# somepago/DCR

Measured on AMD Instinct MI355X. Metric: sd21_256px_finetune_imgs_per_sec, higher is better.
Workload: dtype bf16; 1 GPU; model=sd2.1-unet-865M-random-init, global_batch=16, resolution=256, seq_len=77, parallelism=dp1, optimizer=fused_adamw

## Files before the change

### dcr_amd/ops/adamw.py

```python
from __future__ import annotations

from typing import Iterable, List, Tuple

import torch

from . import use_hip, require_hip, count_dispatch

QBLOCK = 256
FP8_MAX = 448.0
STATE_FORMAT = {"state_bits": 8, "qblock": QBLOCK, "codec": "e4m3fn_absmax",
                "second_moment": "sqrt"}


def _nblocks(numel: int) -> int:
    return (numel + QBLOCK - 1) // QBLOCK


def _sqrt_rn(x: torch.Tensor) -> torch.Tensor:
    return x.double().sqrt().float()


@torch.no_grad()
def quantize_blockwise(x: torch.Tensor) -> Tuple[torch.Tensor, torch.Tensor]:
    dev = x.device
    x = x.detach().reshape(-1).float()
    nb = _nblocks(x.numel())
    xp = torch.zeros(nb * QBLOCK, dtype=torch.float32, device=dev)
    xp[: x.numel()] = x
    xp = xp.view(nb, QBLOCK)
    absmax = xp.abs().amax(dim=1)
    scale = torch.full_like(absmax, FP8_MAX).div(absmax)
    ok = torch.isfinite(scale)
    scale = torch.where(ok, scale, torch.zeros_like(scale))
    y = (xp * scale[:, None]).clamp_(-FP8_MAX, FP8_MAX)
# ... 76 lines not shown
            n = p.numel()
            sl = self.flat_param[offset : offset + n]
            gl = self.flat_grad[offset : offset + n]
            if (p.data.dim() == 4 and not p.data.is_contiguous()
                    and p.data.is_contiguous(
                        memory_format=torch.channels_last)):
                K, C, Hh, Ww = p.data.shape
                sl.copy_(p.data.permute(0, 2, 3, 1).reshape(-1))
                p.data = sl.view(K, Hh, Ww, C).permute(0, 3, 1, 2)
                self._grad_views.append(
                    gl.view(K, Hh, Ww, C).permute(0, 3, 1, 2))
            else:
                sl.copy_(p.data.reshape(-1))
                p.data = sl.view_as(p.data)
                self._grad_views.append(gl.view_as(p.data))
            self.offsets.append(offset)
            offset += n
        self.numel = total
        self._view_of = {id(p): v for p, v in zip(self.params, self._grad_views)}
        self._gathered: set = set()
        if self.master is not None:
            self.master.copy_(self.flat_param.float())

        self.hyper = None
        if device_state and device.type == "cuda":
            self.hyper = torch.tensor([lr, 1, 1, 1, 1, 1, 0, 0],
                                      dtype=torch.float32, device=device)

    def zero_grad(self, set_to_none: bool = False):
        if len(self._gathered) != len(self.params):
            self.flat_grad.zero_()
            self._skipped_zero = False
        else:
            self._skipped_zero = True
        self._gathered.clear()
        for p in self.params:
            p.grad = None

    def _ensure_cold_slices(self):
        if not getattr(self, "_skipped_zero", False):
            return
        if len(self._gathered) == len(self.params):
            return
        stale = [self._view_of[id(p)] for p in self.params
                 if id(p) not in self._gathered]
        if stale:
            torch._foreach_zero_(stale)
        self._skipped_zero = False

    @torch.no_grad()
    def gather_grads(self, params=None):
        copy_d, copy_s, add_d, add_s = [], [], [], []
        for p in (params if params is not None else self.params):
            g = p.grad
            if g is None:
                continue
            view = self._view_of[id(p)]
            if g.dtype != view.dtype:
                g = g.to(view.dtype)
            if id(p) in self._gathered:
                add_d.append(view)
                add_s.append(g)
            else:
                copy_d.append(view)
                copy_s.append(g)
                self._gathered.add(id(p))
            p.grad = None
        if copy_d:
            torch._foreach_copy_(copy_d, copy_s)
        if add_d:
            torch._foreach_add_(add_d, add_s)

    @torch.no_grad()
    def step(self, lr: float | None = None):
        self.gather_grads()
        self._ensure_cold_slices()
        if lr is not None:
            self.lr = lr
        self.step_count += 1
        t = self.step_count
        if self.state_bits == 8:
            self._step8(t)
            return
        if use_hip(self.flat_param):
            m = require_hip("adamw")
            if m is not None:
                count_dispatch('adamw')
                if self.master is not None:
                    m.adamw_step_bf16(
                        self.flat_param, self.flat_grad, self.master,
                        self.exp_avg, self.exp_avg_sq, self.lr, self.beta1,
# ... 67 lines not shown
            ts = (self.exp_avg, self.exp_avg_sq)
        return sum(t.numel() * t.element_size() for t in ts)

    @torch.no_grad()
    def step_dev(self, lr: float | None = None):
        assert self.hyper is not None, "built without device_state=True"
        self.gather_grads()
        self._ensure_cold_slices()
        if lr is not None and lr != self.lr:
            self.lr = lr
            self.hyper[0].fill_(lr)
        self.step_count += 1
        m = require_hip("adamw")
        count_dispatch('adamw_dev')
        m.adamw_step_dev(self.flat_param, self.flat_grad, self.master,
                         self.exp_avg, self.exp_avg_sq, self.hyper,
                         self.beta1, self.beta2, self.eps, self.weight_decay,
                         self.max_grad_norm)

    @torch.no_grad()
    def clip_grad_norm_(self, max_norm: float) -> torch.Tensor:
        self.gather_grads()
        self._ensure_cold_slices()
        norm = torch.linalg.vector_norm(self.flat_grad, dtype=torch.float32)
        scale = max_norm / (norm + 1e-6)
        if float(norm) > max_norm:
            self.flat_grad.mul_(scale.to(self.flat_grad.dtype))
        return norm

    def state_dict(self):
        if self.state_bits == 8:
            d = {
                "step": self.step_count,
                "lr": self.lr,
                "flat_param": self.flat_param,
                "exp_avg_q": self.exp_avg_q,
                "exp_avg_absmax": self.exp_avg_absmax,
                "exp_avg_sq_q": self.exp_avg_sq_q,
                "exp_avg_sq_absmax": self.exp_avg_sq_absmax,
                "format": dict(STATE_FORMAT),
            }
            if self.master is not None:
                d["master"] = self.master
            return d
        d = {
            "step": self.step_count,
            "lr": self.lr,
            "exp_avg": self.exp_avg,
            "exp_avg_sq": self.exp_avg_sq,
            "flat_param": self.flat_param,
        }
# ... 81 lines not shown
```

### dcr_amd/ops/build.py

```python
from __future__ import annotations

import os
import shutil
from pathlib import Path

HERE = Path(__file__).resolve().parent
HIP_DIR = HERE / "hip"
BUILD_DIR = HERE / "_build"
TARGET = HERE / "_dcr_hip.so"

SOURCES = [
    HIP_DIR / "bindings.cpp",
    HIP_DIR / "norms.hip",
    HIP_DIR / "norms_nhwc.hip",
    HIP_DIR / "elementwise.hip",
    HIP_DIR / "reduce.hip",
    HIP_DIR / "adamw8.hip",
    HIP_DIR / "attention.hip",
    HIP_DIR / "conv_nhwc.hip",
    HIP_DIR / "conv_nhwc_bwd.hip",
    HIP_DIR / "gemm.hip",
    HIP_DIR / "maxsim.hip",
    HIP_DIR / "splitsim.hip",
    HIP_DIR / "topk_sim.hip",
]


def build_extension(verbose: bool = False, force: bool = False) -> Path:
    os.environ.setdefault("PYTORCH_ROCM_ARCH", "gfx950")
    os.environ.setdefault("MAX_JOBS", str(min(16, os.cpu_count() or 4)))
    from torch.utils import cpp_extension

    BUILD_DIR.mkdir(parents=True, exist_ok=True)
    if force:
        for f in BUILD_DIR.glob("*"):
            if f.is_file():
                f.unlink()

    cpp_extension.load(
        name="_dcr_hip",
        sources=[str(s) for s in SOURCES],
        build_directory=str(BUILD_DIR),
        extra_cflags=["-O3"],
        extra_cuda_cflags=["-O3"],
# ... 14 lines not shown
```

### dcr_amd/ops/hip/bindings.cpp

```cpp

#include <torch/extension.h>
#include <ATen/cuda/CUDAContext.h>

#include <climits>
#include <cstdint>
#include <limits>

#include "dcr_launchers.h"

using namespace dcr;

namespace {

DType dtype_of(const at::Tensor& t) {
  switch (t.scalar_type()) {
    case at::kFloat: return DT_F32;
    case at::kHalf: return DT_F16;
    case at::kBFloat16: return DT_BF16;
    default: TORCH_CHECK(false, "dcr_hip: unsupported dtype ", t.scalar_type());
  }
}

hipStream_t cur_stream() {
  return at::cuda::getCurrentCUDAStream().stream();
}

at::Tensor as_f32(const at::Tensor& t) {
  return t.scalar_type() == at::kFloat ? t.contiguous()
                                       : t.to(at::kFloat).contiguous();
// ... 225 lines not shown

void adamw_step(at::Tensor p, at::Tensor g, at::Tensor m, at::Tensor v,
                double lr, double beta1, double beta2, double eps, double wd,
                int64_t step) {
  TORCH_CHECK(p.is_cuda() && p.scalar_type() == at::kFloat,
              "adamw: fp32 flat params expected");
  TORCH_CHECK(p.is_contiguous() && g.is_contiguous() && m.is_contiguous() &&
              v.is_contiguous());
  adamw_launch(p.data_ptr<float>(), g.data_ptr<float>(), m.data_ptr<float>(),
               v.data_ptr<float>(), p.numel(), (float)lr, (float)beta1,
               (float)beta2, (float)eps, (float)wd, step, cur_stream());
}

void adamw_step_bf16(at::Tensor p, at::Tensor g, at::Tensor master,
                     at::Tensor m, at::Tensor v, double lr, double beta1,
                     double beta2, double eps, double wd, int64_t step) {
  TORCH_CHECK(p.is_cuda() && p.scalar_type() == at::kBFloat16);
  TORCH_CHECK(master.scalar_type() == at::kFloat);
  TORCH_CHECK(p.is_contiguous() && g.is_contiguous() && master.is_contiguous());
  adamw_bf16_launch(p.data_ptr(), g.data_ptr(), master.data_ptr<float>(),
                    m.data_ptr<float>(), v.data_ptr<float>(), p.numel(),
                    (float)lr, (float)beta1, (float)beta2, (float)eps,
                    (float)wd, step, cur_stream());
}

void adamw_step_dev(at::Tensor p, at::Tensor g, c10::optional<at::Tensor> master,
                    at::Tensor m, at::Tensor v, at::Tensor hyper, double beta1,
                    double beta2, double eps, double wd, double max_norm) {
  TORCH_CHECK(hyper.is_cuda() && hyper.scalar_type() == at::kFloat &&
              hyper.numel() == 8 && hyper.is_contiguous());
  TORCH_CHECK(p.is_contiguous() && g.is_contiguous());
  const bool bf16 = p.scalar_type() == at::kBFloat16;
  float* mp = nullptr;
  if (bf16) {
    TORCH_CHECK(master.has_value() && master->scalar_type() == at::kFloat,
                "bf16 device-state adamw needs the fp32 master");
    mp = master->data_ptr<float>();
  } else {
    TORCH_CHECK(p.scalar_type() == at::kFloat);
  }
  adamw_dev_launch(bf16 ? 1 : 0, p.data_ptr(), g.data_ptr(), mp,
                   m.data_ptr<float>(), v.data_ptr<float>(), p.numel(),
                   (float)beta1, (float)beta2, (float)eps, (float)wd,
                   (float)max_norm, hyper.data_ptr<float>(), cur_stream());
}

// ... 684 lines not shown
  mod.def("attn_fwd_d512", &attn_fwd_d512);
  mod.def("attn_bwd_gen", &attn_bwd_gen);
  mod.def("attn_fwd_v2", &attn_fwd_v2);
  mod.def("attn_fwd_v3", &attn_fwd_v3);
  mod.def("attn_fwd_v4", &attn_fwd_v4);
  mod.def("attn_bwd", &attn_bwd);
  mod.def("attn_bwd_v4", &attn_bwd_v4);
  mod.def("mfma_probe", &mfma_probe);
  mod.def("groupnorm_silu_fwd", &groupnorm_silu_fwd);
  mod.def("groupnorm_silu_bwd", &groupnorm_silu_bwd);
  mod.def("groupnorm_silu_nhwc_fwd", &groupnorm_silu_nhwc_fwd);
  mod.def("groupnorm_silu_nhwc_bwd", &groupnorm_silu_nhwc_bwd);
  mod.def("layernorm_fwd", &layernorm_fwd);
  mod.def("layernorm_bwd", &layernorm_bwd, py::arg("dy"), py::arg("x"),
          py::arg("w"), py::arg("mean"), py::arg("rstd"),
          py::arg("blocks") = 0);
  mod.def("colsum", &colsum);
  mod.def("colsum_grouped", &colsum_grouped);
  mod.def("geglu_fwd", &geglu_fwd);
  mod.def("geglu_bwd", &geglu_bwd);
  mod.def("adamw_step", &adamw_step);
  mod.def("adamw_step_bf16", &adamw_step_bf16);
  mod.def("adamw_step_dev", &adamw_step_dev);
  mod.def("adamw8_step", &adamw8_step, py::arg("p"), py::arg("g"),
          py::arg("exp_avg_q"), py::arg("exp_avg_absmax"),
          py::arg("exp_avg_sq_q"), py::arg("exp_avg_sq_absmax"), py::arg("lr"),
          py::arg("beta1"), py::arg("beta2"), py::arg("eps"), py::arg("wd"),
          py::arg("step"));
  mod.def("adamw8_step_bf16", &adamw8_step_bf16, py::arg("p"), py::arg("g"),
          py::arg("master"), py::arg("exp_avg_q"), py::arg("exp_avg_absmax"),
          py::arg("exp_avg_sq_q"), py::arg("exp_avg_sq_absmax"), py::arg("lr"),
          py::arg("beta1"), py::arg("beta2"), py::arg("eps"), py::arg("wd"),
          py::arg("step"));
  mod.def("add_noise", &add_noise);
  mod.def("get_velocity", &get_velocity);
  mod.def("cfg_combine", &cfg_combine);
  mod.def("lincomb", &lincomb);
}
```

### dcr_amd/ops/hip/dcr_launchers.h

```cpp
#pragma once

#include <hip/hip_runtime.h>

namespace dcr {

enum DType { DT_F32 = 0, DT_F16 = 1, DT_BF16 = 2 };

void gn_fwd_launch(DType dt, const void* x, const void* w, const void* b,
                   bool w_f32, void* y, float* mean, float* rstd, int NG,
                   int G, int Cg, int HW, float eps, bool silu, hipStream_t s);
void gn_bwd_launch(DType dt, const void* dy, const void* x, const void* w,
                   const void* b, bool w_f32, const float* mean,
                   const float* rstd, void* dx, float* dw, float* db, int NG,
                   int G, int Cg, int HW, bool silu, hipStream_t s);
void ln_fwd_launch(DType dt, const void* x, const void* w, const void* b,
                   bool w_f32, void* y, float* mean, float* rstd, long M,
                   int N, float eps, hipStream_t s);
void ln_bwd_launch(DType dt, const void* dy, const void* x, const void* w,
                   bool w_f32, const float* mean, const float* rstd, void* dx,
                   float* dw, float* db, long M, int N, hipStream_t s);
int ln_bwd_v2_blocks(long M, int N);
void ln_bwd_v2_launch(DType dt, const void* dy, const void* x, const void* w,
                      bool w_f32, const float* mean, const float* rstd,
                      void* dx, float* slab, void* dwdb, int blocks, long M,
// ... 5 lines not shown
                        int N, int R, int C, int G, float eps, bool silu,
                        hipStream_t s);
void gn_nhwc_bwd_launch(DType dt, const void* dy, const void* x, const void* w,
                        const void* b, bool w_f32, const float* mean,
                        const float* rstd, float* ws, void* dx, void* dwdb,
                        int N, int R, int C, int G, bool silu,
                        hipStream_t s);

int colsum_chunks(int dt, long groups, long rows_per_group, int C, int cap);
void colsum_launch(DType dt, const void* x, float* slab, void* out_n, void* out,
                   long groups, long rows_per_group, int C, int chunks,
                   hipStream_t s);

void geglu_fwd_launch(DType dt, const void* x, void* y, long M, long N,
                      hipStream_t s);
void geglu_bwd_launch(DType dt, const void* dy, const void* x, void* dx,
                      long M, long N, hipStream_t s);
void adamw_launch(float* p, const float* g, float* m, float* v, long n,
                  float lr, float b1, float b2, float eps, float wd, long step,
                  hipStream_t s);
void adamw_bf16_launch(void* p, const void* g, float* master, float* m,
                       float* v, long n, float lr, float b1, float b2,
                       float eps, float wd, long step, hipStream_t s);
void adamw_dev_launch(int bf16, void* p, const void* g, float* master,
                      float* m, float* v, long n, float b1, float b2,
                      float eps, float wd, float max_norm, float* hyper,
                      hipStream_t s);
void adamw8_launch(int bf16, void* p, const void* g, float* master,
                   unsigned char* mq, float* mabs, unsigned char* rq,
                   float* rabs, long n, double lr, double b1, double b2,
                   double eps, double wd, long step, hipStream_t s);
void sched_launch(DType dt, int mode, const void* x0, const void* noise,
                  const float* ac, const long* t, void* out, long per_sample,
                  long total, hipStream_t s);
void cfg_launch(DType dt, const void* eu, const void* et, void* out, float s_,
                long total, hipStream_t s);
void lincomb_launch(DType dt, const void* X, const void* Y, const void* Z,
                    void* out, float a, float b, float c, long total,
                    hipStream_t s);

void attn_fwd_launch(const void* q, const void* k, const void* v, void* o,
                     float* lse, int BH, int Lq, int Lk, int H, float scale,
                     bool causal, hipStream_t s);
void attn_fwd_v2_launch(const void* q, const void* k, const void* v, void* o,
                        float* lse, int BH, int Lq, int Lk, int H, float scale,
                        bool causal, hipStream_t s);
// ... 75 lines not shown
```

### dcr_amd/ops/hip/elementwise.hip

```cpp

#include "dcr_common.h"

using namespace dcr;

template <typename T>
__global__ void geglu_fwd_kernel(const T* __restrict__ x, T* __restrict__ y,
                                 long M, long N) {
  const long nvec = M * N / 4;
  for (long i = (long)blockIdx.x * blockDim.x + threadIdx.x; i < nvec;
       i += (long)gridDim.x * blockDim.x) {
    long e = i * 4;
    long row = e / N, col = e % N;
    const T* base = x + row * 2 * N;
    f32x4 a = load4<T>(base + col);
    f32x4 g = load4<T>(base + N + col);
    f32x4 o;
    o.x = a.x * gelu_erf(g.x);
    o.y = a.y * gelu_erf(g.y);
    o.z = a.z * gelu_erf(g.z);
    o.w = a.w * gelu_erf(g.w);
    store4<T>(y + row * N + col, o);
  }
}

template <typename T>
__global__ void geglu_bwd_kernel(const T* __restrict__ dy, const T* __restrict__ x,
                                 T* __restrict__ dx, long M, long N) {
  const long nvec = M * N / 4;
  for (long i = (long)blockIdx.x * blockDim.x + threadIdx.x; i < nvec;
       i += (long)gridDim.x * blockDim.x) {
    long e = i * 4;
    long row = e / N, col = e % N;
    const T* base = x + row * 2 * N;
    T* dbase = dx + row * 2 * N;
    f32x4 a = load4<T>(base + col);
    f32x4 g = load4<T>(base + N + col);
    f32x4 d = load4<T>(dy + row * N + col);
    f32x4 da, dg;
    da.x = d.x * gelu_erf(g.x); dg.x = d.x * a.x * dgelu_erf(g.x);
    da.y = d.y * gelu_erf(g.y); dg.y = d.y * a.y * dgelu_erf(g.y);
    da.z = d.z * gelu_erf(g.z); dg.z = d.z * a.z * dgelu_erf(g.z);
    da.w = d.w * gelu_erf(g.w); dg.w = d.w * a.w * dgelu_erf(g.w);
    store4<T>(dbase + col, da);
    store4<T>(dbase + N + col, dg);
  }
}

__global__ void adamw_kernel(float* __restrict__ p, const float* __restrict__ g,
                             float* __restrict__ m, float* __restrict__ v,
                             long n, float lr, float beta1, float beta2,
                             float eps, float wd, float inv_bc1, float inv_bc2) {
  const long nvec = n / 4;
  for (long i = (long)blockIdx.x * blockDim.x + threadIdx.x; i < nvec;
       i += (long)gridDim.x * blockDim.x) {
    long e = i * 4;
    f32x4 pv = load4<float>(p + e);
    f32x4 gv = load4<float>(g + e);
    f32x4 mv = load4<float>(m + e);
    f32x4 vv = load4<float>(v + e);
#pragma unroll
    for (int k = 0; k < 4; ++k) {
      float gg = (&gv.x)[k];
      float mm = beta1 * (&mv.x)[k] + (1.f - beta1) * gg;
      float vvk = beta2 * (&vv.x)[k] + (1.f - beta2) * gg * gg;
      (&mv.x)[k] = mm;
      (&vv.x)[k] = vvk;
      float denom = sqrtf(vvk * inv_bc2) + eps;
      float upd = (mm * inv_bc1) / denom + wd * (&pv.x)[k];
      (&pv.x)[k] -= lr * upd;
    }
    store4<float>(p + e, pv);
    store4<float>(m + e, mv);
    store4<float>(v + e, vv);
  }
  long tail = nvec * 4 + (long)blockIdx.x * blockDim.x + threadIdx.x;
  if (tail < n) {
    float gg = g[tail];
    float mm = beta1 * m[tail] + (1.f - beta1) * gg;
    float vvk = beta2 * v[tail] + (1.f - beta2) * gg * gg;
    m[tail] = mm; v[tail] = vvk;
    float denom = sqrtf(vvk * inv_bc2) + eps;
    p[tail] -= lr * ((mm * inv_bc1) / denom + wd * p[tail]);
  }
}

__global__ void adamw_bf16_kernel(__hip_bfloat16* __restrict__ p,
                                  const __hip_bfloat16* __restrict__ g,
                                  float* __restrict__ master,
                                  float* __restrict__ m, float* __restrict__ v,
                                  long n, float lr, float beta1, float beta2,
                                  float eps, float wd, float inv_bc1,
                                  float inv_bc2) {
  const long nvec = n / 4;
  for (long i = (long)blockIdx.x * blockDim.x + threadIdx.x; i < nvec;
       i += (long)gridDim.x * blockDim.x) {
    long e = i * 4;
    f32x4 gv = load4<__hip_bfloat16>(g + e);
    f32x4 pv = load4<float>(master + e);
    f32x4 mv = load4<float>(m + e);
    f32x4 vv = load4<float>(v + e);
#pragma unroll
    for (int kk = 0; kk < 4; ++kk) {
      float gg = (&gv.x)[kk];
      float mm = beta1 * (&mv.x)[kk] + (1.f - beta1) * gg;
      float vvk = beta2 * (&vv.x)[kk] + (1.f - beta2) * gg * gg;
      (&mv.x)[kk] = mm;
      (&vv.x)[kk] = vvk;
      float denom = sqrtf(vvk * inv_bc2) + eps;
      (&pv.x)[kk] -= lr * ((mm * inv_bc1) / denom + wd * (&pv.x)[kk]);
    }
    store4<float>(master + e, pv);
    store4<float>(m + e, mv);
    store4<float>(v + e, vv);
    store4<__hip_bfloat16>(p + e, pv);
  }
  long tail = nvec * 4 + (long)blockIdx.x * blockDim.x + threadIdx.x;
  if (tail < n) {
    float gg = to_f32<__hip_bfloat16>(g[tail]);
    float mm = beta1 * m[tail] + (1.f - beta1) * gg;
    float vvk = beta2 * v[tail] + (1.f - beta2) * gg * gg;
    m[tail] = mm; v[tail] = vvk;
    float denom = sqrtf(vvk * inv_bc2) + eps;
    float pv = master[tail] - lr * ((mm * inv_bc1) / denom + wd * master[tail]);
    master[tail] = pv;
    p[tail] = from_f32<__hip_bfloat16>(pv);
  }
}

template <typename T, int MODE>
__global__ void sched_kernel(const T* __restrict__ x0, const T* __restrict__ noise,
                             const float* __restrict__ ac, const long* __restrict__ t,
                             T* __restrict__ out, long per_sample, long total) {
  const long nvec = total / 4;
  for (long i = (long)blockIdx.x * blockDim.x + threadIdx.x; i < nvec;
       i += (long)gridDim.x * blockDim.x) {
    long e = i * 4;
    long bidx = e / per_sample;
    float a = ac[t[bidx]];
    float sa = sqrtf(a), sb = sqrtf(1.f - a);
    f32x4 xa = load4<T>(x0 + e);
    f32x4 xb = load4<T>(noise + e);
// ... 206 lines not shown
  switch (dt) {
    case DT_F32: hipLaunchKernelGGL((geglu_fwd_kernel<float>), grid, block, 0, s, (const float*)x, (float*)y, M, N); break;
    case DT_F16: hipLaunchKernelGGL((geglu_fwd_kernel<__half>), grid, block, 0, s, (const __half*)x, (__half*)y, M, N); break;
    case DT_BF16: hipLaunchKernelGGL((geglu_fwd_kernel<__hip_bfloat16>), grid, block, 0, s, (const __hip_bfloat16*)x, (__hip_bfloat16*)y, M, N); break;
  }
}

void geglu_bwd_launch(DType dt, const void* dy, const void* x, void* dx,
                      long M, long N, hipStream_t s) {
  dim3 grid(ew_blocks(M * N / 4)), block(256);
  switch (dt) {
    case DT_F32: hipLaunchKernelGGL((geglu_bwd_kernel<float>), grid, block, 0, s, (const float*)dy, (const float*)x, (float*)dx, M, N); break;
    case DT_F16: hipLaunchKernelGGL((geglu_bwd_kernel<__half>), grid, block, 0, s, (const __half*)dy, (const __half*)x, (__half*)dx, M, N); break;
    case DT_BF16: hipLaunchKernelGGL((geglu_bwd_kernel<__hip_bfloat16>), grid, block, 0, s, (const __hip_bfloat16*)dy, (const __hip_bfloat16*)x, (__hip_bfloat16*)dx, M, N); break;
  }
}

void adamw_launch(float* p, const float* g, float* m, float* v, long n,
                  float lr, float b1, float b2, float eps, float wd, long step,
                  hipStream_t s) {
  float bc1 = 1.f - powf(b1, (float)step);
  float bc2 = 1.f - powf(b2, (float)step);
  dim3 grid(ew_blocks(n / 4)), block(256);
  hipLaunchKernelGGL(adamw_kernel, grid, block, 0, s, p, g, m, v, n, lr, b1, b2,
                     eps, wd, 1.f / bc1, 1.f / bc2);
}

void adamw_bf16_launch(void* p, const void* g, float* master, float* m,
                       float* v, long n, float lr, float b1, float b2,
                       float eps, float wd, long step, hipStream_t s) {
  float bc1 = 1.f - powf(b1, (float)step);
  float bc2 = 1.f - powf(b2, (float)step);
  dim3 grid(ew_blocks(n / 4)), block(256);
  hipLaunchKernelGGL(adamw_bf16_kernel, grid, block, 0, s,
                     (__hip_bfloat16*)p, (const __hip_bfloat16*)g, master, m, v,
                     n, lr, b1, b2, eps, wd, 1.f / bc1, 1.f / bc2);
}

void adamw_dev_launch(int bf16, void* p, const void* g, float* master,
                      float* m, float* v, long n, float b1, float b2,
                      float eps, float wd, float max_norm, float* hyper,
                      hipStream_t s) {
  dim3 grid(ew_blocks(n / 4)), block(256);
  if (bf16)
    hipLaunchKernelGGL((gnormsq_kernel<__hip_bfloat16>), grid, block, 0, s,
                       (const __hip_bfloat16*)g, n, hyper + 6);
  else
    hipLaunchKernelGGL((gnormsq_kernel<float>), grid, block, 0, s,
                       (const float*)g, n, hyper + 6);
  hipLaunchKernelGGL(adamw_prologue_kernel, dim3(1), dim3(1), 0, s, hyper,
                     b1, b2, max_norm);
  if (bf16)
    hipLaunchKernelGGL(adamw_bf16_dev_kernel, grid, block, 0, s,
                       (__hip_bfloat16*)p, (const __hip_bfloat16*)g, master,
                       m, v, n, b1, b2, eps, wd, hyper);
  else
    hipLaunchKernelGGL(adamw_dev_kernel, grid, block, 0, s, (float*)p,
                       (const float*)g, m, v, n, b1, b2, eps, wd, hyper);
}
// ... 53 lines not shown
```

### dcr_amd/parallel/ddp.py

```python
from __future__ import annotations

from typing import List, Optional

import torch.distributed as dist

from ..ops.adamw import FusedAdamW
from . import dist as dist_utils


class _Bucket:
    __slots__ = ("start", "end", "params", "pending", "work")

    def __init__(self, start: int, end: int, params: list):
        self.start = start
        self.end = end
        self.params = params
        self.pending = len(params)
        self.work = None


class GradBucketAllReduce:

    def __init__(self, optimizer: FusedAdamW, bucket_mb: float = 64.0,
                 process_group: Optional[object] = None):
# ... 19 lines not shown
        for p, off in reversed(runs):
            n = p.numel()
            if cur_start is None:
                cur_params, cur_start, cur_end = [p], off, off + n
            else:
                cur_params.append(p)
                cur_start = off
            if cur_end - cur_start >= bucket_elems:
                self._push_bucket(cur_start, cur_end, cur_params)
                cur_params, cur_start, cur_end = [], None, None
        if cur_params:
            self._push_bucket(cur_start, cur_end, cur_params)

        for p in self.opt.params:
            p.register_post_accumulate_grad_hook(self._hook)

    def _push_bucket(self, start, end, params):
        b = _Bucket(start, end, list(params))
        self.buckets.append(b)
        for p in params:
            self._param_bucket[id(p)] = b

    def _launch(self, b: _Bucket):
        self.opt.gather_grads(b.params)
        sl = self.opt.flat_grad[b.start:b.end]
        b.work = dist.all_reduce(sl, group=self.pg, async_op=True)

    def _hook(self, param):
        if not self.require_backward_grad_sync:
            return
        b = self._param_bucket[id(param)]
        b.pending -= 1
        if b.pending == 0:
            self._launch(b)

    def finalize(self):
        self.opt.gather_grads()
        self.opt._ensure_cold_slices()
        if not self._enabled or not self.require_backward_grad_sync:
            self._reset()
            return
        for b in self.buckets:
            if b.work is None and b.pending > 0:
                self._launch(b)
        launched = any(b.work is not None for b in self.buckets)
        for b in self.buckets:
            if b.work is not None:
                b.work.wait()
        if launched and self.world > 1:
            self.opt.flat_grad.div_(self.world)
        self._reset()

    def _reset(self):
        for b in self.buckets:
            b.pending = len(b.params)
            b.work = None
```

### dcr_amd/train/trainer.py

```python
from __future__ import annotations

import os
import random
import time
from pathlib import Path
from typing import Optional

import numpy as np
import torch
import torch.nn.functional as F
from torch.utils.data import DataLoader, WeightedRandomSampler
from torch.utils.data.distributed import DistributedSampler

from ..data import (HashTokenizer, ObjectAttributeDataset, SyntheticImageDataset,
                    collate_fn, load_tokenizer)
from ..models import (AutoencoderKL, CLIPTextModel, UNet2DConditionModel,
                      UNetConfig, model_configs)
from ..models.model_io import save_pipeline_index
from ..ops.adamw import FusedAdamW
from ..parallel import GradBucketAllReduce, dist as dist_utils
from ..schedulers import DDPMScheduler
from ..utils import Tracker
from ..utils.profiler import PhaseProfiler
from .config import TrainConfig, get_lr
# ... 275 lines not shown

            if self.noise_scheduler.prediction_type == "epsilon":
                target = noise
            elif self.noise_scheduler.prediction_type == "v_prediction":
                target = self.noise_scheduler.get_velocity(latents, noise, timesteps)
            else:
                raise ValueError(self.noise_scheduler.prediction_type)

        loss = F.mse_loss(model_pred.float(), target.float(), reduction="mean")
        accum = cfg.gradient_accumulation_steps
        bwd_loss = loss / accum if accum > 1 else loss
        with self.prof.phase("backward"):
            if self.scaler is not None:
                self.scaler.scale(bwd_loss).backward()
            else:
                bwd_loss.backward()

        if sync_gradients:
            with self.prof.phase("optimizer"):
                self.ddp.finalize()
                grads_finite = True
                if self.scaler is not None:
                    inv = 1.0 / self.scaler.get_scale()
                    self.optimizer.flat_grad.mul_(inv)
                    grads_finite = bool(
                        torch.isfinite(self.optimizer.flat_grad).all())
                if grads_finite:
                    lr_step = get_lr(cfg, self.global_step, self.world)
                    if self.optimizer.hyper is not None:
                        self.optimizer.step_dev(lr=lr_step)
                    else:
                        self.optimizer.clip_grad_norm_(cfg.max_grad_norm)
                        self.optimizer.step(lr=lr_step)
                    if self.scaler is not None:
                        self._finite_streak += 1
                        if self._finite_streak >= 2000:
                            self.scaler.update(self.scaler.get_scale() * 2.0)
                            self._finite_streak = 0
                        else:
                            self.scaler.update(self.scaler.get_scale())
                else:
                    self._finite_streak = 0
                    self.scaler.update(self.scaler.get_scale() * 0.5)
                self.optimizer.zero_grad()
            self.global_step += 1
        return loss.detach()

    def fit(self, max_steps: Optional[int] = None, sample_fn=None):
        try:
            self._fit_inner(max_steps, sample_fn)
        except Exception:
            import traceback
            print(f"rank {self.rank}: training failed\n{traceback.format_exc()}",
                  flush=True)
            if dist_utils.is_dist():
                import torch.distributed as dist
# ... 96 lines not shown
```

Baseline: 265.9 imgs/sec.

## Fuse grad gather with sum-of-squares and fold clip coefficient into AdamW

Replaces the per-tensor foreach copy of gradients into the flat arena with one table-driven HIP kernel that also produces per-chunk squared-norm partials. A single-block finalize kernel turns these into the norm and clip coefficient on the device, and new clip-aware AdamW kernels read that coefficient. This removes the separate vector_norm pass, the host sync from float(norm), and the separate scaling multiply. The cost is extra bookkeeping to invalidate cached partials whenever the arena is written, plus a pinned host upload of the offset table on every step.

```diff
diff --git a/dcr_amd/ops/adamw.py b/dcr_amd/ops/adamw.py
--- a/dcr_amd/ops/adamw.py
+++ b/dcr_amd/ops/adamw.py
@@ -1,15 +1,23 @@
 from __future__ import annotations
 
+import os
 from typing import Iterable, List, Tuple
 
 import torch
 
 from . import use_hip, require_hip, count_dispatch
+
+GATHER_CH = 16384
+GATHER_GRID = 0
 
 QBLOCK = 256
 FP8_MAX = 448.0
 STATE_FORMAT = {"state_bits": 8, "qblock": QBLOCK, "codec": "e4m3fn_absmax",
                 "second_moment": "sqrt"}
+
+
+def fused_grad_tail_enabled() -> bool:
+    return os.environ.get("DCR_FUSED_GRAD_TAIL", "1") != "0"
 
 
 def _nblocks(numel: int) -> int:
@@ -132,12 +140,19 @@
         if self.master is not None:
             self.master.copy_(self.flat_param.float())
 
+        self._nvb_all = sum((p.numel() + GATHER_CH - 1) // GATHER_CH
+                            for p in self.params)
+        self._partials = None
+        self._norm_rec = None
+        self._sumsq_valid = False
+
         self.hyper = None
         if device_state and device.type == "cuda":
             self.hyper = torch.tensor([lr, 1, 1, 1, 1, 1, 0, 0],
                                       dtype=torch.float32, device=device)
 
     def zero_grad(self, set_to_none: bool = False):
+        self.arena_written()
         if len(self._gathered) != len(self.params):
             self.flat_grad.zero_()
             self._skipped_zero = False
@@ -155,11 +170,30 @@
         stale = [self._view_of[id(p)] for p in self.params
                  if id(p) not in self._gathered]
         if stale:
+            self.arena_written()
             torch._foreach_zero_(stale)
         self._skipped_zero = False
 
-    @torch.no_grad()
-    def gather_grads(self, params=None):
+    def arena_written(self):
+        self._sumsq_valid = False
+
+    def _native_tail(self):
+        if not self.flat_grad.is_cuda or not fused_grad_tail_enabled():
+            return None
+        if torch.cuda.is_current_stream_capturing():
+            return None
+        return require_hip("grad_tail")
+
+    def _get_partials(self) -> torch.Tensor:
+        if self._partials is None:
+            self._partials = torch.empty(
+                max(self._nvb_all, 1), dtype=torch.float32,
+                device=self.flat_grad.device)
+        return self._partials
+
+    @torch.no_grad()
+    def gather_grads(self, params=None, sumsq: bool = True):
+        m = self._native_tail()
         copy_d, copy_s, add_d, add_s = [], [], [], []
         for p in (params if params is not None else self.params):
             g = p.grad
@@ -176,7 +210,23 @@
                 copy_s.append(g)
                 self._gathered.add(id(p))
             p.grad = None
-        if copy_d:
+        if copy_d or add_d:
+            self.arena_written()
+        if copy_d and m is not None:
+            fused = (sumsq and params is None and not add_d
+                     and len(copy_d) == len(self.params))
+            rejected = m.grad_gather(
+                self.flat_grad, copy_d, copy_s,
+                self._get_partials() if fused else None,
+                GATHER_CH, GATHER_GRID)
+            count_dispatch('grad_gather')
+            for i in rejected:
+                count_dispatch('grad_gather_fallback')
+                copy_d[i].copy_(copy_s[i])
+            self._sumsq_valid = fused and not rejected
+        elif copy_d:
+            if self.flat_grad.is_cuda:
+                count_dispatch('grad_gather_foreach')
             torch._foreach_copy_(copy_d, copy_s)
         if add_d:
             torch._foreach_add_(add_d, add_s)
@@ -290,11 +340,57 @@
     def clip_grad_norm_(self, max_norm: float) -> torch.Tensor:
         self.gather_grads()
         self._ensure_cold_slices()
+        if self.flat_grad.is_cuda:
+            count_dispatch('grad_norm_aten')
         norm = torch.linalg.vector_norm(self.flat_grad, dtype=torch.float32)
         scale = max_norm / (norm + 1e-6)
         if float(norm) > max_norm:
+            self.arena_written()
             self.flat_grad.mul_(scale.to(self.flat_grad.dtype))
         return norm
+
+    def _norm_record(self, m, max_norm: float) -> torch.Tensor:
+        if self._norm_rec is None:
+            self._norm_rec = torch.zeros(3, dtype=torch.float32,
+                                         device=self.flat_grad.device)
+        partials = self._get_partials()
+        if not self._sumsq_valid:
+            count_dispatch('grad_sumsq')
+            m.grad_sumsq(self.flat_grad, self._grad_views, partials,
+                         GATHER_CH, GATHER_GRID)
+            self._sumsq_valid = True
+        count_dispatch('grad_norm_finalize')
+        m.sumsq_finalize(partials, self._nvb_all, float(max_norm),
+                         self._norm_rec)
+        return self._norm_rec
+
+    @torch.no_grad()
+    def clip_and_step(self, max_norm: float, lr: float | None = None) -> torch.Tensor:
+        m = self._native_tail() if self.state_bits == 32 else None
+        if m is None:
+            norm = self.clip_grad_norm_(max_norm)
+            self.step(lr=lr)
+            return norm
+        self.gather_grads()
+        self._ensure_cold_slices()
+        rec = self._norm_record(m, max_norm)
+        if lr is not None:
+            self.lr = lr
+        self.step_count += 1
+        count_dispatch('adamw')
+        count_dispatch('adamw_clip')
+        if self.master is not None:
+            m.adamw_step_bf16_clip(
+                self.flat_param, self.flat_grad, self.master, self.exp_avg,
+                self.exp_avg_sq, self.lr, self.beta1, self.beta2, self.eps,
+                self.weight_decay, self.step_count, rec)
+        else:
+            m.adamw_step_clip(
+                self.flat_param, self.flat_grad, self.exp_avg,
+                self.exp_avg_sq, self.lr, self.beta1, self.beta2, self.eps,
+                self.weight_decay, self.step_count, rec)
+        self.arena_written()
+        return rec[1]
 
     def state_dict(self):
         if self.state_bits == 8:
diff --git a/dcr_amd/ops/build.py b/dcr_amd/ops/build.py
--- a/dcr_amd/ops/build.py
+++ b/dcr_amd/ops/build.py
@@ -20,6 +20,7 @@
     HIP_DIR / "conv_nhwc.hip",
     HIP_DIR / "conv_nhwc_bwd.hip",
     HIP_DIR / "gemm.hip",
+    HIP_DIR / "grad_tail.hip",
     HIP_DIR / "maxsim.hip",
     HIP_DIR / "splitsim.hip",
     HIP_DIR / "topk_sim.hip",
diff --git a/dcr_amd/ops/hip/bindings.cpp b/dcr_amd/ops/hip/bindings.cpp
--- a/dcr_amd/ops/hip/bindings.cpp
+++ b/dcr_amd/ops/hip/bindings.cpp
@@ -4,7 +4,9 @@
 
 #include <climits>
 #include <cstdint>
+#include <cstring>
 #include <limits>
+#include <vector>
 
 #include "dcr_launchers.h"
 
@@ -276,6 +278,170 @@
                     m.data_ptr<float>(), v.data_ptr<float>(), p.numel(),
                     (float)lr, (float)beta1, (float)beta2, (float)eps,
                     (float)wd, step, cur_stream());
+}
+
+namespace {
+
+void gt_check_arena(const at::Tensor& arena, int64_t ch) {
+  TORCH_CHECK(arena.is_cuda() && arena.dim() == 1 && arena.is_contiguous(),
+              "grad tail: the arena must be a flat contiguous GPU tensor");
+  TORCH_CHECK(arena.scalar_type() == at::kBFloat16 ||
+              arena.scalar_type() == at::kFloat,
+              "grad tail: bf16 or fp32 arena expected");
+  TORCH_CHECK(ch >= 8 && ch % 8 == 0 && ch <= (1 << 24),
+              "grad tail: chunk must be a multiple of 8 elements, got ", ch);
+}
+
+int64_t gt_view_offset(const at::Tensor& arena, const at::Tensor& view) {
+  TORCH_CHECK(view.scalar_type() == arena.scalar_type() &&
+              view.device() == arena.device() &&
+              view.is_non_overlapping_and_dense(),
+              "grad tail: not a dense view of the arena");
+  const int64_t es = arena.element_size();
+  const int64_t byte_off = (const char*)view.data_ptr() - (const char*)arena.data_ptr();
+  TORCH_CHECK(byte_off >= 0 && byte_off % es == 0 &&
+              byte_off / es + view.numel() <= arena.numel(),
+              "grad tail: view outside the arena");
+  return byte_off / es;
+}
+
+bool gt_qualifies(const at::Tensor& g, const at::Tensor& view) {
+  if (!g.defined() || g.device() != view.device() ||
+      g.scalar_type() != view.scalar_type() || g.sizes() != view.sizes() ||
+      !g.is_non_overlapping_and_dense())
+    return false;
+  for (int64_t d = 0; d < g.dim(); ++d)
+    if (g.size(d) > 1 && g.stride(d) != view.stride(d)) return false;
+  return reinterpret_cast<uintptr_t>(g.data_ptr()) % g.element_size() == 0;
+}
+
+at::Tensor gt_upload(const at::Tensor& arena, const std::vector<int64_t>& rows) {
+  auto host = at::empty({(int64_t)rows.size()},
+                        at::TensorOptions().dtype(at::kLong).pinned_memory(true));
+  std::memcpy(host.data_ptr<int64_t>(), rows.data(), rows.size() * sizeof(int64_t));
+  auto dev = at::empty({(int64_t)rows.size()}, arena.options().dtype(at::kLong));
+  dev.copy_(host, true);
+  return dev;
+}
+
+float* gt_partials(const c10::optional<at::Tensor>& partials,
+                   const at::Tensor& arena, int64_t nvb) {
+  if (!partials.has_value()) return nullptr;
+  TORCH_CHECK(partials->is_cuda() && partials->device() == arena.device() &&
+              partials->scalar_type() == at::kFloat &&
+              partials->is_contiguous() && partials->numel() >= nvb,
+              "grad tail: partials must hold ", nvb, " floats on the GPU");
+  return partials->data_ptr<float>();
+}
+
+}
+
+std::vector<int64_t> grad_gather(at::Tensor arena, std::vector<at::Tensor> views,
+                                 std::vector<at::Tensor> grads,
+                                 c10::optional<at::Tensor> partials,
+                                 int64_t ch, int64_t grid) {
+  gt_check_arena(arena, ch);
+  TORCH_CHECK(views.size() == grads.size(), "grad_gather: list lengths differ");
+  std::vector<int64_t> rows, rejected;
+  rows.reserve(4 * views.size());
+  int64_t nvb = 0;
+  for (size_t i = 0; i < views.size(); ++i) {
+    if (!gt_qualifies(grads[i], views[i])) {
+      rejected.push_back((int64_t)i);
+      continue;
+    }
+    const int64_t n = views[i].numel();
+    if (n == 0) continue;
+    const int64_t off = gt_view_offset(arena, views[i]);
+    rows.push_back((int64_t)reinterpret_cast<uintptr_t>(grads[i].data_ptr()));
+    rows.push_back(off);
+    rows.push_back(n);
+    rows.push_back(nvb);
+    nvb += (n + ch - 1) / ch;
+  }
+  if (rows.empty()) return rejected;
+  float* pp = gt_partials(partials, arena, nvb);
+  auto table = gt_upload(arena, rows);
+  grad_gather_launch(dtype_of(arena), (const long*)table.data_ptr<int64_t>(),
+                     (int)(rows.size() / 4), nvb, arena.data_ptr(), pp, (int)ch,
+                     grad_gather_grid(nvb, (int)grid), true,
+                     cur_stream());
+  return rejected;
+}
+
+int64_t grad_sumsq(at::Tensor arena, std::vector<at::Tensor> views,
+                   at::Tensor partials, int64_t ch, int64_t grid) {
+  gt_check_arena(arena, ch);
+  std::vector<int64_t> rows;
+  rows.reserve(4 * views.size());
+  int64_t nvb = 0;
+  for (const auto& v : views) {
+    const int64_t n = v.numel();
+    if (n == 0) continue;
+    const int64_t off = gt_view_offset(arena, v);
+    rows.push_back((int64_t)reinterpret_cast<uintptr_t>(
+        (const char*)arena.data_ptr() + off * arena.element_size()));
+    rows.push_back(off);
+    rows.push_back(n);
+    rows.push_back(nvb);
+    nvb += (n + ch - 1) / ch;
+  }
+  float* pp = gt_partials(partials, arena, nvb);
+  if (rows.empty()) return 0;
+  auto table = gt_upload(arena, rows);
+  grad_gather_launch(dtype_of(arena), (const long*)table.data_ptr<int64_t>(),
+                     (int)(rows.size() / 4), nvb, arena.data_ptr(), pp, (int)ch,
+                     grad_gather_grid(nvb, (int)grid), false,
+                     cur_stream());
+  return nvb;
+}
+
+void sumsq_finalize(at::Tensor partials, int64_t nvb, double max_norm,
+                    at::Tensor rec) {
+  TORCH_CHECK(partials.is_cuda() && partials.scalar_type() == at::kFloat &&
+              partials.is_contiguous() && nvb >= 0 && partials.numel() >= nvb,
+              "sumsq_finalize: partials must hold nvb floats on the GPU");
+  TORCH_CHECK(rec.is_cuda() && rec.scalar_type() == at::kFloat &&
+              rec.is_contiguous() && rec.numel() == 3,
+              "sumsq_finalize: rec must be float[3] on the GPU");
+  sumsq_finalize_launch(partials.data_ptr<float>(), nvb, (float)max_norm,
+                        rec.data_ptr<float>(), cur_stream());
+}
+
+static void gt_check_rec(const at::Tensor& rec, const at::Tensor& p) {
+  TORCH_CHECK(rec.is_cuda() && rec.device() == p.device() &&
+              rec.scalar_type() == at::kFloat && rec.is_contiguous() &&
+              rec.numel() == 3, "adamw_clip: rec must be float[3] on the GPU");
+}
+
+void adamw_step_clip(at::Tensor p, at::Tensor g, at::Tensor m, at::Tensor v,
+                     double lr, double beta1, double beta2, double eps,
+                     double wd, int64_t step, at::Tensor rec) {
+  TORCH_CHECK(p.is_cuda() && p.scalar_type() == at::kFloat &&
+              g.scalar_type() == at::kFloat && g.numel() == p.numel(),
+              "adamw_clip: fp32 flat params and grads expected");
+  TORCH_CHECK(p.is_contiguous() && g.is_contiguous() && m.is_contiguous() &&
+              v.is_contiguous());
+  gt_check_rec(rec, p);
+  adamw_clip_launch(p.data_ptr<float>(), g.data_ptr<float>(),
+                    m.data_ptr<float>(), v.data_ptr<float>(), p.numel(),
+                    (float)lr, (float)beta1, (float)beta2, (float)eps,
+                    (float)wd, step, rec.data_ptr<float>(), cur_stream());
+}
+
+void adamw_step_bf16_clip(at::Tensor p, at::Tensor g, at::Tensor master,
+                          at::Tensor m, at::Tensor v, double lr, double beta1,
+                          double beta2, double eps, double wd, int64_t step,
+                          at::Tensor rec) {
+  TORCH_CHECK(p.is_cuda() && p.scalar_type() == at::kBFloat16 &&
+              g.scalar_type() == at::kBFloat16 && g.numel() == p.numel());
+  TORCH_CHECK(master.scalar_type() == at::kFloat);
+  TORCH_CHECK(p.is_contiguous() && g.is_contiguous() && master.is_contiguous());
+  gt_check_rec(rec, p);
+  adamw_bf16_clip_launch(p.data_ptr(), g.data_ptr(), master.data_ptr<float>(),
+                         m.data_ptr<float>(), v.data_ptr<float>(), p.numel(),
+                         (float)lr, (float)beta1, (float)beta2, (float)eps,
+                         (float)wd, step, rec.data_ptr<float>(), cur_stream());
 }
 
 void adamw_step_dev(at::Tensor p, at::Tensor g, c10::optional<at::Tensor> master,
@@ -1006,6 +1172,14 @@
   mod.def("adamw_step", &adamw_step);
   mod.def("adamw_step_bf16", &adamw_step_bf16);
   mod.def("adamw_step_dev", &adamw_step_dev);
+  mod.def("adamw_step_clip", &adamw_step_clip);
+  mod.def("adamw_step_bf16_clip", &adamw_step_bf16_clip);
+  mod.def("grad_gather", &grad_gather, py::arg("arena"), py::arg("views"),
+          py::arg("grads"), py::arg("partials") = py::none(),
+          py::arg("ch") = 16384, py::arg("grid") = 0);
+  mod.def("grad_sumsq", &grad_sumsq, py::arg("arena"), py::arg("views"),
+          py::arg("partials"), py::arg("ch") = 16384, py::arg("grid") = 0);
+  mod.def("sumsq_finalize", &sumsq_finalize);
   mod.def("adamw8_step", &adamw8_step, py::arg("p"), py::arg("g"),
           py::arg("exp_avg_q"), py::arg("exp_avg_absmax"),
           py::arg("exp_avg_sq_q"), py::arg("exp_avg_sq_absmax"), py::arg("lr"),
diff --git a/dcr_amd/ops/hip/dcr_launchers.h b/dcr_amd/ops/hip/dcr_launchers.h
--- a/dcr_amd/ops/hip/dcr_launchers.h
+++ b/dcr_amd/ops/hip/dcr_launchers.h
@@ -51,6 +51,19 @@
 void adamw_bf16_launch(void* p, const void* g, float* master, float* m,
                        float* v, long n, float lr, float b1, float b2,
                        float eps, float wd, long step, hipStream_t s);
+void adamw_clip_launch(float* p, float* g, float* m, float* v, long n,
+                       float lr, float b1, float b2, float eps, float wd,
+                       long step, const float* rec, hipStream_t s);
+void adamw_bf16_clip_launch(void* p, void* g, float* master, float* m,
+                            float* v, long n, float lr, float b1, float b2,
+                            float eps, float wd, long step, const float* rec,
+                            hipStream_t s);
+int grad_gather_grid(long nvb, int grid_req);
+void grad_gather_launch(DType dt, const long* table, int nparams, long nvb,
+                        void* arena, float* partials, int ch, int grid,
+                        bool store, hipStream_t s);
+void sumsq_finalize_launch(const float* partials, long nvb, float max_norm,
+                           float* rec, hipStream_t s);
 void adamw_dev_launch(int bf16, void* p, const void* g, float* master,
                       float* m, float* v, long n, float b1, float b2,
                       float eps, float wd, float max_norm, float* hyper,
diff --git a/dcr_amd/ops/hip/elementwise.hip b/dcr_amd/ops/hip/elementwise.hip
--- a/dcr_amd/ops/hip/elementwise.hip
+++ b/dcr_amd/ops/hip/elementwise.hip
@@ -46,10 +46,14 @@
   }
 }
 
-__global__ void adamw_kernel(float* __restrict__ p, const float* __restrict__ g,
+template <bool CLIP>
+__global__ void adamw_kernel(float* __restrict__ p, float* __restrict__ g,
                              float* __restrict__ m, float* __restrict__ v,
                              long n, float lr, float beta1, float beta2,
-                             float eps, float wd, float inv_bc1, float inv_bc2) {
+                             float eps, float wd, float inv_bc1, float inv_bc2,
+                             const float* __restrict__ rec) {
+  const float coef = CLIP ? rec[2] : 1.f;
+  const bool clip = CLIP && coef != 1.f;
   const long nvec = n / 4;
   for (long i = (long)blockIdx.x * blockDim.x + threadIdx.x; i < nvec;
        i += (long)gridDim.x * blockDim.x) {
@@ -58,6 +62,10 @@
     f32x4 gv = load4<float>(g + e);
     f32x4 mv = load4<float>(m + e);
     f32x4 vv = load4<float>(v + e);
+    if (clip) {
+      gv.x *= coef; gv.y *= coef; gv.z *= coef; gv.w *= coef;
+      store4<float>(g + e, gv);
+    }
 #pragma unroll
     for (int k = 0; k < 4; ++k) {
       float gg = (&gv.x)[k];
@@ -76,6 +84,7 @@
   long tail = nvec * 4 + (long)blockIdx.x * blockDim.x + threadIdx.x;
   if (tail < n) {
     float gg = g[tail];
+    if (clip) { gg *= coef; g[tail] = gg; }
     float mm = beta1 * m[tail] + (1.f - beta1) * gg;
     float vvk = beta2 * v[tail] + (1.f - beta2) * gg * gg;
     m[tail] = mm; v[tail] = vvk;
@@ -84,18 +93,29 @@
   }
 }
 
+template <bool CLIP>
 __global__ void adamw_bf16_kernel(__hip_bfloat16* __restrict__ p,
-                                  const __hip_bfloat16* __restrict__ g,
+                                  __hip_bfloat16* __restrict__ g,
                                   float* __restrict__ master,
                                   float* __restrict__ m, float* __restrict__ v,
                                   long n, float lr, float beta1, float beta2,
                                   float eps, float wd, float inv_bc1,
-                                  float inv_bc2) {
+                                  float inv_bc2, const float* __restrict__ rec) {
+  const float coef = CLIP ? rec[2] : 1.f;
+  const bool clip = CLIP && coef != 1.f;
+  const float cb = to_f32<__hip_bfloat16>(from_f32<__hip_bfloat16>(coef));
   const long nvec = n / 4;
   for (long i = (long)blockIdx.x * blockDim.x + threadIdx.x; i < nvec;
        i += (long)gridDim.x * blockDim.x) {
     long e = i * 4;
     f32x4 gv = load4<__hip_bfloat16>(g + e);
+    if (clip) {
+#pragma unroll
+      for (int kk = 0; kk < 4; ++kk)
+        (&gv.x)[kk] = to_f32<__hip_bfloat16>(
+            from_f32<__hip_bfloat16>((&gv.x)[kk] * cb));
+      store4<__hip_bfloat16>(g + e, gv);
+    }
     f32x4 pv = load4<float>(master + e);
     f32x4 mv = load4<float>(m + e);
     f32x4 vv = load4<float>(v + e);
@@ -117,6 +137,11 @@
   long tail = nvec * 4 + (long)blockIdx.x * blockDim.x + threadIdx.x;
   if (tail < n) {
     float gg = to_f32<__hip_bfloat16>(g[tail]);
+    if (clip) {
+      __hip_bfloat16 gb = from_f32<__hip_bfloat16>(gg * cb);
+      g[tail] = gb;
+      gg = to_f32<__hip_bfloat16>(gb);
+    }
     float mm = beta1 * m[tail] + (1.f - beta1) * gg;
     float vvk = beta2 * v[tail] + (1.f - beta2) * gg * gg;
     m[tail] = mm; v[tail] = vvk;
@@ -369,8 +394,19 @@
   float bc1 = 1.f - powf(b1, (float)step);
   float bc2 = 1.f - powf(b2, (float)step);
   dim3 grid(ew_blocks(n / 4)), block(256);
-  hipLaunchKernelGGL(adamw_kernel, grid, block, 0, s, p, g, m, v, n, lr, b1, b2,
-                     eps, wd, 1.f / bc1, 1.f / bc2);
+  hipLaunchKernelGGL(adamw_kernel<false>, grid, block, 0, s, p,
+                     const_cast<float*>(g), m, v, n, lr, b1, b2, eps, wd,
+                     1.f / bc1, 1.f / bc2, (const float*)nullptr);
+}
+
+void adamw_clip_launch(float* p, float* g, float* m, float* v, long n,
+                       float lr, float b1, float b2, float eps, float wd,
+                       long step, const float* rec, hipStream_t s) {
+  float bc1 = 1.f - powf(b1, (float)step);
+  float bc2 = 1.f - powf(b2, (float)step);
+  dim3 grid(ew_blocks(n / 4)), block(256);
+  hipLaunchKernelGGL(adamw_kernel<true>, grid, block, 0, s, p, g, m, v, n, lr,
+                     b1, b2, eps, wd, 1.f / bc1, 1.f / bc2, rec);
 }
 
 void adamw_bf16_launch(void* p, const void* g, float* master, float* m,
@@ -379,9 +415,22 @@
   float bc1 = 1.f - powf(b1, (float)step);
   float bc2 = 1.f - powf(b2, (float)step);
   dim3 grid(ew_blocks(n / 4)), block(256);
-  hipLaunchKernelGGL(adamw_bf16_kernel, grid, block, 0, s,
-                     (__hip_bfloat16*)p, (const __hip_bfloat16*)g, master, m, v,
-                     n, lr, b1, b2, eps, wd, 1.f / bc1, 1.f / bc2);
+  hipLaunchKernelGGL(adamw_bf16_kernel<false>, grid, block, 0, s,
+                     (__hip_bfloat16*)p, (__hip_bfloat16*)const_cast<void*>(g),
+                     master, m, v, n, lr, b1, b2, eps, wd, 1.f / bc1,
+                     1.f / bc2, (const float*)nullptr);
+}
+
+void adamw_bf16_clip_launch(void* p, void* g, float* master, float* m,
+                            float* v, long n, float lr, float b1, float b2,
+                            float eps, float wd, long step, const float* rec,
+                            hipStream_t s) {
+  float bc1 = 1.f - powf(b1, (float)step);
+  float bc2 = 1.f - powf(b2, (float)step);
+  dim3 grid(ew_blocks(n / 4)), block(256);
+  hipLaunchKernelGGL(adamw_bf16_kernel<true>, grid, block, 0, s,
+                     (__hip_bfloat16*)p, (__hip_bfloat16*)g, master, m, v, n,
+                     lr, b1, b2, eps, wd, 1.f / bc1, 1.f / bc2, rec);
 }
 
 void adamw_dev_launch(int bf16, void* p, const void* g, float* master,
diff --git a/dcr_amd/ops/hip/grad_tail.hip b/dcr_amd/ops/hip/grad_tail.hip
--- /dev/null
+++ b/dcr_amd/ops/hip/grad_tail.hip
@@ -0,0 +1,230 @@
+
+#include <cstdint>
+
+#include "dcr_common.h"
+#include "dcr_launchers.h"
+
+using namespace dcr;
+
+#define GT_THREADS 256
+#define GT_UNROLL 4
+
+template <int W>
+__device__ __forceinline__ uint4 gt_load16(const char* __restrict__ p) {
+  uint4 r;
+  if (W == 16) {
+    r = *reinterpret_cast<const uint4*>(p);
+  } else if (W == 8) {
+    uint2 a = reinterpret_cast<const uint2*>(p)[0];
+    uint2 b = reinterpret_cast<const uint2*>(p)[1];
+    r = make_uint4(a.x, a.y, b.x, b.y);
+  } else if (W == 4) {
+    const unsigned* q = reinterpret_cast<const unsigned*>(p);
+    r = make_uint4(q[0], q[1], q[2], q[3]);
+  } else {
+    const unsigned short* q = reinterpret_cast<const unsigned short*>(p);
+    r = make_uint4((unsigned)q[0] | ((unsigned)q[1] << 16),
+                   (unsigned)q[2] | ((unsigned)q[3] << 16),
+                   (unsigned)q[4] | ((unsigned)q[5] << 16),
+                   (unsigned)q[6] | ((unsigned)q[7] << 16));
+  }
+  return r;
+}
+
+template <typename T>
+__device__ __forceinline__ float gt_group_sumsq(uint4 v);
+
+template <>
+__device__ __forceinline__ float gt_group_sumsq<float>(uint4 v) {
+#pragma clang fp contract(off)
+  float a = __uint_as_float(v.x), b = __uint_as_float(v.y);
+  float c = __uint_as_float(v.z), d = __uint_as_float(v.w);
+  return (a * a + b * b) + (c * c + d * d);
+}
+
+template <>
+__device__ __forceinline__ float gt_group_sumsq<__hip_bfloat16>(uint4 v) {
+#pragma clang fp contract(off)
+  float q[4];
+#pragma unroll
+  for (int k = 0; k < 4; ++k) {
+    unsigned w = (&v.x)[k];
+    float lo = __uint_as_float(w << 16);
+    float hi = __uint_as_float(w & 0xffff0000u);
+    q[k] = lo * lo + hi * hi;
+  }
+  return (q[0] + q[1]) + (q[2] + q[3]);
+}
+
+template <typename T, int W, bool SUMSQ, bool STORE>
+__device__ __forceinline__ float gt_body(const T* __restrict__ src,
+                                         T* __restrict__ dst, int ng, float s) {
+#pragma clang fp contract(off)
+  constexpr int G = 16 / sizeof(T);
+  int g = threadIdx.x;
+  for (; g + (GT_UNROLL - 1) * GT_THREADS < ng; g += GT_UNROLL * GT_THREADS) {
+    uint4 v[GT_UNROLL];
+#pragma unroll
+    for (int u = 0; u < GT_UNROLL; ++u)
+      v[u] = gt_load16<W>(reinterpret_cast<const char*>(
+          src + (long)(g + u * GT_THREADS) * G));
+    if (STORE) {
+#pragma unroll
+      for (int u = 0; u < GT_UNROLL; ++u)
+        *reinterpret_cast<uint4*>(dst + (long)(g + u * GT_THREADS) * G) = v[u];
+    }
+    if (SUMSQ) {
+#pragma unroll
+      for (int u = 0; u < GT_UNROLL; ++u) s = s + gt_group_sumsq<T>(v[u]);
+    }
+  }
+  for (; g < ng; g += GT_THREADS) {
+    uint4 v = gt_load16<W>(reinterpret_cast<const char*>(src + (long)g * G));
+    if (STORE) *reinterpret_cast<uint4*>(dst + (long)g * G) = v;
+    if (SUMSQ) s = s + gt_group_sumsq<T>(v);
+  }
+  return s;
+}
+
+template <typename T, bool SUMSQ, bool STORE>
+__global__ __launch_bounds__(GT_THREADS)
+void grad_gather_kernel(const long* __restrict__ table, int nparams, long nvb,
+                        T* __restrict__ arena, float* __restrict__ partials,
+                        int ch) {
+  __shared__ float lds[2 * GT_THREADS / DCR_WAVE];
+  constexpr int G = 16 / sizeof(T);
+  const int t = threadIdx.x;
+  for (long vb = blockIdx.x; vb < nvb; vb += gridDim.x) {
+    int lo = 0, hi = nparams - 1;
+    while (lo < hi) {
+      int mid = (lo + hi + 1) >> 1;
+      if (table[4 * mid + 3] <= vb) lo = mid; else hi = mid - 1;
+    }
+    const long* row = table + 4 * lo;
+    const long n = row[2];
+    const long e0 = (vb - row[3]) * (long)ch;
+    const long left = n - e0;
+    const int len = left < (long)ch ? (int)left : ch;
+    const T* src = reinterpret_cast<const T*>(row[0]) + e0;
+    T* dst = arena + row[1] + e0;
+
+    int h = (int)(((16u - (unsigned)(reinterpret_cast<uintptr_t>(dst) & 15u)) & 15u)
+                  / sizeof(T));
+    if (h > len) h = len;
+    const int ng = (len - h) / G;
+    const int r = len - h - ng * G;
+
+    float s = 0.f;
+    if (t < h) {
+#pragma clang fp contract(off)
+      T x = src[t];
+      if (STORE) dst[t] = x;
+      float f = to_f32<T>(x);
+      if (SUMSQ) s = f * f;
+    }
+    const unsigned d = (unsigned)(reinterpret_cast<uintptr_t>(src) -
+                                  reinterpret_cast<uintptr_t>(dst));
+    const T* bs = src + h;
+    T* bd = dst + h;
+    if ((d & 15u) == 0)
+      s = gt_body<T, 16, SUMSQ, STORE>(bs, bd, ng, s);
+    else if ((d & 7u) == 0)
+      s = gt_body<T, 8, SUMSQ, STORE>(bs, bd, ng, s);
+    else if ((d & 3u) == 0)
+      s = gt_body<T, 4, SUMSQ, STORE>(bs, bd, ng, s);
+    else
+      s = gt_body<T, sizeof(T) < 4 ? 2 : 4, SUMSQ, STORE>(bs, bd, ng, s);
+    if (t < r) {
+#pragma clang fp contract(off)
+      const int i = h + ng * G + t;
+      T x = src[i];
+      if (STORE) dst[i] = x;
+      float f = to_f32<T>(x);
+      if (SUMSQ) s = s + f * f;
+    }
+    if (SUMSQ) {
+      float2 tot = block_reduce_sum2(s, 0.f, lds);
+      if (t == 0) partials[vb] = tot.x;
+    }
+  }
+}
+
+#define GT_FIN_THREADS 1024
+__global__ __launch_bounds__(GT_FIN_THREADS)
+void sumsq_finalize_kernel(const float* __restrict__ partials, long nvb,
+                           float max_norm, float* __restrict__ rec) {
+  __shared__ double sh[GT_FIN_THREADS];
+  const int t = threadIdx.x;
+  double a = 0.0;
+  long i = t;
+  for (; i + 7L * GT_FIN_THREADS < nvb; i += 8L * GT_FIN_THREADS) {
+    float v[8];
+#pragma unroll
+    for (int u = 0; u < 8; ++u) v[u] = partials[i + (long)u * GT_FIN_THREADS];
+#pragma unroll
+    for (int u = 0; u < 8; ++u) a += (double)v[u];
+  }
+  for (; i < nvb; i += GT_FIN_THREADS) a += (double)partials[i];
+  sh[t] = a;
+  __syncthreads();
+  for (int off = GT_FIN_THREADS / 2; off > 0; off >>= 1) {
+    if (t < off) sh[t] += sh[t + off];
+    __syncthreads();
+  }
+  if (t == 0) {
+#pragma clang fp contract(off)
+    const float ss = (float)sh[0];
+    const float norm = sqrtf(ss);
+    float coef = 1.f;
+    if (norm > max_norm) coef = (1.f / (norm + 1e-6f)) * max_norm;
+    rec[0] = ss;
+    rec[1] = norm;
+    rec[2] = coef;
+  }
+}
+
+namespace dcr {
+
+int grad_gather_grid(long nvb, int grid_req) {
+  long g = grid_req > 0 ? grid_req : 8192;
+  if (g > nvb) g = nvb;
+  if (g < 1) g = 1;
+  return (int)g;
+}
+
+template <typename T>
+static void gather_dispatch(const long* table, int nparams, long nvb, void* arena,
+                            float* partials, int ch, int grid, bool store,
+                            hipStream_t s) {
+  dim3 gr(grid), bl(GT_THREADS);
+  T* a = (T*)arena;
+  if (store && partials)
+    hipLaunchKernelGGL((grad_gather_kernel<T, true, true>), gr, bl, 0, s, table,
+                       nparams, nvb, a, partials, ch);
+  else if (store)
+    hipLaunchKernelGGL((grad_gather_kernel<T, false, true>), gr, bl, 0, s, table,
+                       nparams, nvb, a, partials, ch);
+  else
+    hipLaunchKernelGGL((grad_gather_kernel<T, true, false>), gr, bl, 0, s, table,
+                       nparams, nvb, a, partials, ch);
+}
+
+void grad_gather_launch(DType dt, const long* table, int nparams, long nvb,
+                        void* arena, float* partials, int ch, int grid,
+                        bool store, hipStream_t s) {
+  if (nvb <= 0 || nparams <= 0) return;
+  if (dt == DT_BF16)
+    gather_dispatch<__hip_bfloat16>(table, nparams, nvb, arena, partials, ch,
+                                    grid, store, s);
+  else
+    gather_dispatch<float>(table, nparams, nvb, arena, partials, ch, grid,
+                           store, s);
+}
+
+void sumsq_finalize_launch(const float* partials, long nvb, float max_norm,
+                           float* rec, hipStream_t s) {
+  hipLaunchKernelGGL(sumsq_finalize_kernel, dim3(1), dim3(GT_FIN_THREADS), 0, s,
+                     partials, nvb, max_norm, rec);
+}
+
+}
diff --git a/dcr_amd/parallel/ddp.py b/dcr_amd/parallel/ddp.py
--- a/dcr_amd/parallel/ddp.py
+++ b/dcr_amd/parallel/ddp.py
@@ -65,7 +65,8 @@
             self._param_bucket[id(p)] = b
 
     def _launch(self, b: _Bucket):
-        self.opt.gather_grads(b.params)
+        self.opt.gather_grads(b.params, sumsq=False)
+        self.opt.arena_written()
         sl = self.opt.flat_grad[b.start:b.end]
         b.work = dist.all_reduce(sl, group=self.pg, async_op=True)
 
@@ -91,6 +92,7 @@
             if b.work is not None:
                 b.work.wait()
         if launched and self.world > 1:
+            self.opt.arena_written()
             self.opt.flat_grad.div_(self.world)
         self._reset()
 
diff --git a/dcr_amd/train/trainer.py b/dcr_amd/train/trainer.py
--- a/dcr_amd/train/trainer.py
+++ b/dcr_amd/train/trainer.py
@@ -321,6 +321,7 @@
                 grads_finite = True
                 if self.scaler is not None:
                     inv = 1.0 / self.scaler.get_scale()
+                    self.optimizer.arena_written()
                     self.optimizer.flat_grad.mul_(inv)
                     grads_finite = bool(
                         torch.isfinite(self.optimizer.flat_grad).all())
@@ -329,8 +330,8 @@
                     if self.optimizer.hyper is not None:
                         self.optimizer.step_dev(lr=lr_step)
                     else:
-                        self.optimizer.clip_grad_norm_(cfg.max_grad_norm)
-                        self.optimizer.step(lr=lr_step)
+                        self.optimizer.clip_and_step(cfg.max_grad_norm,
+                                                     lr=lr_step)
                     if self.scaler is not None:
                         self._finite_streak += 1
                         if self._finite_streak >= 2000:
```

Result: faster. 280.7 imgs/sec, median of 6 (+5.5%).
